# shaohua-pan/RobustCap

Measured on AMD Instinct MI355X. Metric: body-frames/sec (sig_mp fwd + FK) at batch 256, higher is better.
Workload: dtype f32; 1 GPU; synthetic 60 fps, 6 IMU + 33 keypoints, batch 256 x 1448 frames per GPU (256 bodies in total, weak scaling), confidence schedule 'mixed', seeded random weights (63.4 M params); batch_per_gpu=256, bodies_total=256, frames=1448, conf=mixed, parallelism=dp1 (sequence sharding)

## Files before the change

### robustcap_amd/csrc/rc_api.cpp

```cpp
#include "../../include/robustcap_hip.h"
#include "rc_ctx.h"

#include <algorithm>
#include <cstdio>
#include <cstdlib>
#include <cstring>
#include <map>
#include <string>
#include <thread>
#include <vector>

#define RC_SPLIT_MIN_BATCH 48
#define RC_TILE64_MIN_BATCH 192

#ifndef RC_NC1280
#define RC_NC1280 10
#endif

static thread_local std::string g_create_error;

int fail(rc_ctx* ctx, int code, const std::string& msg) {
    if (ctx) ctx->err = msg; else g_create_error = msg;
    return code;
}
// ... 152 lines not shown
    p.nt = (c->live_nt_mask >> s.net) & 1u;
    return p;
}
GemmProblem lstm_problem(const rc_ctx* c, const Stage& s, int layer) {
    const NetDev& n = c->net[s.net];
    const long long BH = (long long)c->Bp * n.H;
    GemmProblem p{};
    if (layer == 0) p.seg[0] = seg(n.x1, n.H, n.H);
    else p.seg[0] = seg(n.h, n.H, n.H, RC_PAR_DST, BH);
    p.seg[1] = seg(n.h + layer * RC_HBUF * BH, n.H, n.H, RC_PAR_SRC, BH);
    p.W = n.Wl[layer]; p.Ws = n.Wls[layer]; p.bias = n.bl[layer];
    p.hstate = n.h + layer * RC_HBUF * BH; p.cstate = n.c + layer * (long long)c->B * n.H; p.h_par_stride = BH; p.H = n.H;
    p.steps = n.steps; p.flags = s.flags ? s.flags : c->fb.flags; p.flag_bit = s.flag_bit;
    p.epi = RC_EPI_LSTM;
    int mr, nc;
    pick_tile(n.H, s.rows_hint < 0 ? c->B : s.rows_hint, &mr, &nc);
    if (s.rows_hint < 0 && c->B >= RC_TILE64_MIN_BATCH) {
        if (s.net == N6 && c->tile6[0]) { mr = c->tile6[0]; nc = c->tile6[1]; }
        if ((s.net == N3 || s.net == N7 || s.net == N8) && c->tile378[0]) { mr = c->tile378[0]; nc = c->tile378[1]; }
        if (s.net == N2 && c->tile2[0]) { mr = c->tile2[0]; nc = c->tile2[1]; }
        if (s.net == N4 && c->tile4[0]) { mr = c->tile4[0]; nc = c->tile4[1]; }
    }
    const int rows = s.rows_hint < 0 ? c->B : (s.rows_hint < c->B ? s.rows_hint : c->B);
    if (lds_problem(c, rows)) { mr = 16; nc = 8; }
    p.n_tiles = n.H / (4 * nc); p.m_tiles = (rows + 16 * mr - 1) / (16 * mr); p.Kp = 2 * n.H; p.nc = nc; p.mr = mr;
    p.nt = (c->live_nt_mask >> s.net) & 1u;
    return p;
}
GemmProblem lin2_problem(const rc_ctx* c, const Stage& s) {
    const NetDev& n = c->net[s.net];
    const long long BH = (long long)c->Bp * n.H;
    GemmProblem p = dense_problem(c, n.lin2, seg(n.h + RC_HBUF * BH, n.H, 0, RC_PAR_DST, BH), s.y, false, s.flag_bit,
                                  s.flags ? s.flags : c->fb.flags, n.steps, false);
    p.out_flags = c->fb.flags; p.out_bit = s.out_bit;
    p.nt = 1;
    return p;
}

const int kLdsRegions = 12;

int ensure_lds_pool(rc_ctx* ctx) {
    if (ctx->lds_slab) return RC_OK;
    const size_t m_tiles = ((size_t)ctx->B + 255) / 256;
    const size_t tiles = 320 * m_tiles;
    HIP_TRY(ctx, rc_alloc(ctx->lds_slab, (size_t)kLdsRegions * tiles * RC_LDS_SLAB_FLOATS));
    HIP_TRY(ctx, rc_alloc(ctx->lds_tickets, (size_t)kLdsRegions * tiles));
    HIP_TRY(ctx, hipMemset(ctx->lds_tickets.get(), 0, (size_t)kLdsRegions * tiles * sizeof(int)));
    ctx->lds_region_tiles = tiles;
    return RC_OK;
}

bool timing_pair(rc_ctx* ctx, hipEvent_t* a, hipEvent_t* b) {
    if (ctx->ev_used == ctx->ev_pool.size()) {
        std::pair<HipEvent, HipEvent> ev;
        if (hipEventCreate(rc_out(ev.first)) != hipSuccess || hipEventCreate(rc_out(ev.second)) != hipSuccess) return false;
        ctx->ev_pool.push_back(std::move(ev));
    }
    const auto& ev = ctx->ev_pool[ctx->ev_used++];
    *a = ev.first.get(); *b = ev.second.get();
    return true;
}

int build_lds_problems(rc_ctx* ctx, const std::vector<GemmProblem>& ps, const unsigned char* flags_override, float* slab, int* tickets,
                       LdsProblem* out, int max_p, int* items, size_t* tiles_out, bool resident_order) {
    std::vector<GemmProblem> ord(ps);
    auto key = [&](const GemmProblem& g) -> int {
        if (g.epi == RC_EPI_LSTM) return (resident_order && g.H == 512) ? 0 : g.Kp;
        return 1;
    };
    std::stable_sort(ord.begin(), ord.end(), [&](const GemmProblem& a, const GemmProblem& b) { return key(a) > key(b); });
    if ((int)ord.size() > max_p) return 0;
    int base = 0;
    size_t tiles = 0;
    for (size_t i = 0; i < ord.size(); ++i) {
        const GemmProblem& g = ord[i];
        LdsProblem& p = out[i];
        p = LdsProblem{};
        p.seg[0] = g.seg[0]; p.seg[1] = g.seg[1];
        p.Ws = g.Ws; p.bias = g.bias; p.hstate = g.hstate; p.cstate = g.cstate; p.steps = g.steps;
        p.flags = flags_override ? flags_override : g.flags; p.flag_bit = g.flag_bit;
        p.h_par_stride = g.h_par_stride; p.H = g.H; p.step_off = g.step_off;
        p.m_tiles = g.m_tiles; p.Qs = g.Kp / 32;
        p.epi = g.epi;
        if (g.epi == RC_EPI_LSTM) {
            p.n_tiles = g.H / 32;
            p.ksplit = ctx->lds_ksplit[g.H == 512 ? 0 : (g.H == 1024 ? 1 : 2)];
        } else {
            const long long half = (long long)(g.Kp / 32) * 256;
            p.seg[0].K = g.Kp / 2;
            p.seg[1] = p.seg[0]; p.seg[1].base = g.seg[0].base + half;
            p.alt[0] = g.alt_base; p.alt[1] = g.alt_base ? g.alt_base + half : nullptr;
            p.sel_flags = g.sel_flags; p.sel_bit = g.alt_base ? g.sel_bit : 0;
            p.out = g.out; p.ldo = g.ldo;
            p.n_tiles = g.N / 128;
            p.ksplit = 1;
        }
        p.wg_base = base;
        p.slab = slab + tiles * RC_LDS_SLAB_FLOATS; p.tickets = tickets + tiles;
        tiles += (size_t)p.n_tiles * p.m_tiles;
        base += round_up(p.n_tiles * p.m_tiles * p.ksplit, 8);
    }
    *items = base; *tiles_out = tiles;
    return (int)ord.size();
}
static void build_lds_launch(rc_ctx* ctx, const std::vector<GemmProblem>& ps, const unsigned char* flags_override, float* slab, int* tickets,
                      LdsLaunch& L, int* items, size_t* tiles_out) {
    L = LdsLaunch{};
    L.B = ctx->B;
    L.n = build_lds_problems(ctx, ps, flags_override, slab, tickets, L.p, RC_LDS_MAXP, items, tiles_out);
}

static int launch_lds(rc_ctx* ctx, const std::vector<GemmProblem>& ps_in, const unsigned char* flags_override, hipStream_t st, hipEvent_t stop, bool* launched) {
    if (int rc = ensure_lds_pool(ctx)) return rc;
    static const int replicate = std::getenv("RC_DBG_REPLICATE") ? std::atoi(std::getenv("RC_DBG_REPLICATE")) : 1;
    std::vector<GemmProblem> ps(ps_in);
    for (int r = 1; r < replicate && (int)ps.size() + (int)ps_in.size() <= RC_LDS_MAXP; ++r) ps.insert(ps.end(), ps_in.begin(), ps_in.end());
    LdsLaunch L{};
    const size_t region = ctx->lds_rot++ % kLdsRegions;
    float* slab = ctx->lds_slab.get() + region * ctx->lds_region_tiles * RC_LDS_SLAB_FLOATS;
    int* tickets = ctx->lds_tickets.get() + region * ctx->lds_region_tiles;
    int base = 0;
    size_t tiles = 0;
    build_lds_launch(ctx, ps, flags_override, slab, tickets, L, &base, &tiles);
    if (tiles > ctx->lds_region_tiles) return fail(ctx, RC_ERR_INVALID, "shared-weight launch: more tiles than its slab region holds");
    ctx->stat_lds_launches += 1;
    if (ctx->timing) {
        hipEvent_t a, b;
        if (!timing_pair(ctx, &a, &b)) return fail(ctx, RC_ERR_HIP, "hipEventCreate");
        HIP_TRY(ctx, hipEventRecord(a, st));
        rc_launch_gemm_lds(L, base, st, stop);
        if (launched && stop) *launched = true;
        HIP_TRY(ctx, hipEventRecord(b, st));
    } else {
        rc_launch_gemm_lds(L, base, st, stop);
        if (launched && stop) *launched = true;
    }
    HIP_TRY(ctx, hipGetLastError());
    return RC_OK;
}

static bool dense_items_selftest_wanted(rc_ctx* ctx, const std::vector<GemmProblem>& ps, hipStream_t st, bool fp32) {
    static const int on = std::getenv("RC_DBG_DENSE_ITEMS") ? std::atoi(std::getenv("RC_DBG_DENSE_ITEMS")) : 0;
    if (!on || !ctx->gemm_split || fp32 || ctx->B > 256 || seq_is_engine_stream(ctx, st) || (int)ps.size() > RC_RES_MAXP) return false;
    for (const GemmProblem& p : ps)
        if (!(p.epi == RC_EPI_RELU && p.out_packed && p.N % 128 == 0 && p.Kp % 128 == 0 && p.out_bit == 0 && p.out_col0 == 0 && p.seg[0].par_mode == 0)) return false;
    return true;
}
static int dense_items_selftest(rc_ctx* ctx, const std::vector<GemmProblem>& ps, const unsigned char* flags_override, hipStream_t st) {
    if (int rc = ensure_lds_pool(ctx)) return rc;
    const int n_ints = 2 + RC_RES_MAXP + 1 + 4;
    DevBuf<ResidentTick> tk_d;
    DevBuf<int> ints_d;
    HIP_TRY(ctx, rc_alloc_all(tk_d, 1, ints_d, n_ints));
    ResidentTick T{};
    std::vector<GemmProblem> q(ps);
    for (GemmProblem& p : q) p.m_tiles = 1;
    size_t tiles = 0;
    T.B = ctx->B;
    T.n = build_lds_problems(ctx, q, flags_override, ctx->lds_slab.get(), ctx->lds_tickets.get(), T.p, RC_RES_MAXP, &T.n_items, &tiles, true);
    for (int i = 0; i < RC_RES_MAXP; ++i) T.dep[i][0] = T.dep[i][1] = -1;
    const int base[2] = {0, T.n_items};
    const size_t Bp = (size_t)ctx->Bp;
    HIP_TRY(ctx, hipStreamSynchronize(st));
    for (const GemmProblem& p : ps) HIP_TRY(ctx, hipMemset(p.out, 0xff, Bp * p.N * sizeof(float)));
    HIP_TRY(ctx, hipMemcpy(tk_d.get(), &T, sizeof(T), hipMemcpyHostToDevice));
    HIP_TRY(ctx, hipMemset(ints_d.get(), 0, n_ints * sizeof(int)));
// ... 209 lines not shown
            const double x[3] = {(double)ctx->mesh_vt_h[3 * (size_t)v] - ctx->jroot_h[0], (double)ctx->mesh_vt_h[3 * (size_t)v + 1] - ctx->jroot_h[1],
                                 (double)ctx->mesh_vt_h[3 * (size_t)v + 2] - ctx->jroot_h[2]};
            for (int j = 0; j < 24; ++j) {
                const double ww = jw * ctx->mesh_w_h[(size_t)v * 24 + j];
                double* a = &acc[((size_t)k * 24 + j) * 4];
                a[0] += ww * x[0]; a[1] += ww * x[1]; a[2] += ww * x[2]; a[3] += ww;
            }
        }
    std::vector<float> kM(acc.begin(), acc.end());
    if (!ctx->mesh_kM) if (int rc = dev_alloc(ctx, &ctx->mesh_kM, (size_t)17 * 24 * 4, false)) return rc;
    HIP_TRY(ctx, hipDeviceSynchronize());
    HIP_TRY(ctx, hipMemcpy(ctx->mesh_kM, kM.data(), kM.size() * sizeof(float), hipMemcpyHostToDevice));
    ctx->fold_dirty = false;
    return RC_OK;
}

}

int check_ready(rc_ctx* ctx) {
    if (!ctx) return RC_ERR_INVALID;
    if (!ctx->have_weights) return fail(ctx, RC_ERR_STATE, "weights not finalized (rc_finalize_weights)");
    if (!ctx->have_body) return fail(ctx, RC_ERR_STATE, "body constants not set (rc_set_body)");
    return RC_OK;
}


const BodyConst* rc_ctx_body(rc_ctx* ctx) { return ctx->have_body ? ctx->body : nullptr; }
int rc_ctx_fail(rc_ctx* ctx, int code, const char* msg) { return fail(ctx, code, msg); }
static SubnetDense subnet_dense(const Dense& d) { return SubnetDense{d.W, d.Ws, d.b, d.K, d.N, d.Kp, d.Np}; }
int rc_ctx_subnet_net(rc_ctx* ctx, int ni, SubnetNet* o) {
    if (!ctx->have_weights) return RC_ERR_STATE;
    const NetDev& n = ctx->net[ni];
    o->lin1 = subnet_dense(n.lin1); o->lin2 = subnet_dense(n.lin2);
    for (int l = 0; l < 2; ++l) { o->Wl[l] = n.Wl[l]; o->Wls[l] = n.Wls[l]; o->bl[l] = n.bl[l]; }
    o->in = n.in; o->H = n.H; o->out = n.out;
    return RC_OK;
}
int rc_ctx_init_net(rc_ctx* ctx, SubnetDense out[3]) {
    if (!ctx->have_weights) return RC_ERR_STATE;
    for (int q = 0; q < 3; ++q) out[q] = subnet_dense(ctx->init[q]);
    return RC_OK;
}
int rc_ctx_net_index(const char* name) { return net_index(name); }
int rc_ctx_gemm_split(rc_ctx* ctx) { return ctx->gemm_split ? 1 : 0; }
long long rc_ctx_weights_epoch(rc_ctx* ctx) { return ctx->weights_epoch; }
SubnetOwner& rc_ctx_subnet(rc_ctx* ctx) { return ctx->subnet; }
SmplifyOwner& rc_ctx_smplify(rc_ctx* ctx) { return ctx->smplify; }
unsigned long long rc_ctx_ign_mask(rc_ctx* ctx) { return ctx->ign_mask; }


extern "C" {

int rc_default_params(int32_t live, rc_params* out) {
    if (!out) return RC_ERR_INVALID;
    std::memset(out, 0, sizeof(*out));
    out->conf_lo = live ? 0.85 : 0.7;
    out->conf_hi = live ? 0.9 : 0.8;
    out->contact_threshold = 0.7f;
    out->distance_threshold = 10.0f;
    out->height_threshold = 0.15f;
    out->tran_filter_num = live ? 0.01 : 0.05;
    out->use_flat_floor = 1; out->use_vision_updater = 1; out->use_imu_updater = 1;
    out->live = live ? 1 : 0;
    out->update_vision_freq = 30;
    out->use_reproj_opt = 0;
    out->smooth = 1.0f;
    return RC_OK;
}

int rc_create(int32_t batch, int32_t live, rc_ctx** out) {
    if (!out || batch < 1 || batch > 65535) return fail(nullptr, RC_ERR_INVALID, "rc_create: bad batch");
    int ndev = 0;
    if (hipGetDeviceCount(&ndev) != hipSuccess || ndev == 0) return fail(nullptr, RC_ERR_HIP, "rc_create: no HIP device");
    rc_ctx* ctx = new rc_ctx();
    ctx->B = batch;
    ctx->Bp = round_up(batch, RC_MT);
    (void)hipGetDevice(&ctx->dev);
    rc_default_params(live, &ctx->prm);
    ctx->gemm_split = tune_env("RC_GEMM_SPLIT", batch >= RC_SPLIT_MIN_BATCH ? 1 : 0) != 0;
    live_create(ctx);
    seq_create(ctx);
    ctx->lds_min_rows = tune_env("RC_LDS_MIN_ROWS", std::min(160, std::max(64, batch / 2)));
    ctx->lds_min_batch = tune_env("RC_LDS_MIN_BATCH", ctx->lds_min_batch);
    ctx->lds_ksplit[0] = tune_env("RC_LDS_KSPLIT_512", 1) == 1 ? 1 : 2;
    ctx->lds_ksplit[1] = tune_env("RC_LDS_KSPLIT_1024", batch <= 160 ? 1 : 2) == 1 ? 1 : 2;
    ctx->lds_ksplit[2] = tune_env("RC_LDS_KSPLIT_1280", 2) == 1 ? 1 : 2;
    ctx->tile4[0] = 4; ctx->tile4[1] = 5;
    ctx->tile6[0] = 4; ctx->tile6[1] = 8;
    ctx->tile378[0] = 4; ctx->tile378[1] = 4;
    tile_env("RC_TILE_RNN6", &ctx->tile6[0], &ctx->tile6[1]);
    tile_env("RC_TILE_S2H512", &ctx->tile378[0], &ctx->tile378[1]);
    tile_env("RC_TILE_RNN2", &ctx->tile2[0], &ctx->tile2[1]);
    tile_env("RC_TILE_RNN4", &ctx->tile4[0], &ctx->tile4[1]);
    const struct { const char* knob; int nc, H; } tiles[4] = {{"RC_TILE_RNN6", ctx->tile6[1], 1024}, {"RC_TILE_S2H512", ctx->tile378[1], 512},
                                                              {"RC_TILE_RNN2", ctx->tile2[1], 512}, {"RC_TILE_RNN4", ctx->tile4[1], 1280}};
    for (const auto& t : tiles)
        if (t.nc > 0 && t.H % (4 * t.nc) != 0) {
            rc_destroy(ctx);
            return fail(nullptr, RC_ERR_INVALID, std::string("rc_create: ") + t.knob + " tile width of " + std::to_string(4 * t.nc) +
                                                 " units does not divide H = " + std::to_string(t.H));
        }
    const size_t B = (size_t)batch, Bp = (size_t)ctx->Bp;
    int rc = RC_OK;
    FrameBuffers& fb = ctx->fb;
#define A(ptr, n) if (!rc) rc = dev_alloc(ctx, &(ptr), (n))
    for (int i = 0; i < 6 && !rc; ++i) {
        NetDev& n = ctx->net[i];
        n.in = kNets[i].in; n.H = kNets[i].H; n.out = kNets[i].out;
        n.mr = 2;
        n.nc = n.H == 1280 ? 10 : (n.H == 1024 ? 8 : 4);
        A(n.h, 2 * RC_HBUF * Bp * n.H); A(n.c, 2 * B * n.H); A(n.steps, B); A(n.x1, Bp * n.H);
        A(n.part, (size_t)(n.H / 4) * RC_LIVE_MAXB * round_up(n.out, 4));
    }
    A(ctx->hid1, Bp * 512); A(ctx->hid2, Bp * 1024); A(ctx->xtmp, Bp * 256);
    A(fb.x2, Bp * 128); A(fb.x3, Bp * 256); A(fb.x4, Bp * 256); A(fb.x6, Bp * 256); A(fb.x78, Bp * 256);
    A(fb.x4l, Bp * 256); A(fb.x6l, Bp * 256); A(fb.xi, Bp * 128);
    A(fb.vr, B * 4); A(fb.pc, B * 4); A(fb.r6d, B * 144); A(fb.contact, B * 2); A(fb.init_out, B * 2048);
    A(fb.flags, B); A(fb.flags2, B); A(fb.pend, B); A(fb.regime, B); A(fb.kconf, B); A(fb.gravity, B * 3);
    A(fb.last_pfoot, B * 6); A(fb.last_tran, B * 3); A(fb.floor, B * 33); A(fb.j_temp, B * 99);
    A(fb.has_last, B); A(fb.n_floor, B); A(fb.first_reach, B); A(fb.uv_count, B); A(fb.trace, B * 8);
    A(ctx->body, 1);
#undef A
    if (rc) { g_create_error = ctx->err; rc_destroy(ctx); return rc; }
    fb.h2 = ctx->net[N2].h; fb.c2 = ctx->net[N2].c; fb.steps2 = ctx->net[N2].steps;
    fb.h2_par_stride = (long long)Bp * 512; fb.h2_layer_stride = (long long)RC_HBUF * Bp * 512; fb.c2_layer_stride = (long long)B * 512;
    std::vector<float> g(B * 3);
    for (size_t b = 0; b < B; ++b) { g[3 * b] = -0.0029f; g[3 * b + 1] = 0.9980f; g[3 * b + 2] = -0.0273f; }
    std::vector<int> ones(B, 1);
    if (hipMemcpy(fb.gravity, g.data(), g.size() * 4, hipMemcpyHostToDevice) != hipSuccess ||
        hipMemcpy(fb.first_reach, ones.data(), B * 4, hipMemcpyHostToDevice) != hipSuccess) {
        g_create_error = "rc_create: hipMemcpy failed"; rc_destroy(ctx); return RC_ERR_HIP;
    }
    *out = ctx;
    return RC_OK;
}

int rc_destroy(rc_ctx* ctx) {
    if (!ctx) return RC_OK;
    rc_live_end(ctx);
    (void)hipDeviceSynchronize();
    delete ctx;
    return RC_OK;
}

const char* rc_last_error(const rc_ctx* ctx) { return ctx ? ctx->err.c_str() : g_create_error.c_str(); }

int rc_get_params(const rc_ctx* ctx, rc_params* out) {
    if (!ctx || !out) return RC_ERR_INVALID;
    *out = ctx->prm;
    return RC_OK;
}
int rc_set_params(rc_ctx* ctx, const rc_params* p) {
    if (!ctx || !p) return RC_ERR_INVALID;
    if (!(p->conf_hi > p->conf_lo) || p->update_vision_freq < 0) return fail(ctx, RC_ERR_INVALID, "rc_set_params: bad range");
    ctx->prm = *p;
    return RC_OK;
}

int rc_load_weight(rc_ctx* ctx, const char* key, const float* host, int64_t numel) {
    if (!ctx || !key || !host || numel <= 0) return RC_ERR_INVALID;
    std::string k(key);
    int64_t want = -1;
    for (int i = 0; i < 6 && want < 0; ++i) {
        const NetSpec& s = kNets[i];
        const std::string p = std::string(s.name) + ".";
        if (k.compare(0, p.size(), p)) continue;
// ... 601 lines not shown
```

### robustcap_amd/csrc/rc_ctx.h

```cpp
#pragma once
#include "../../include/robustcap_hip.h"
#include "rc_internal.h"

#include <map>
#include <string>
#include <utility>
#include <vector>

struct NetSpec { const char* name; int in, H, out; };
const NetSpec kNets[6] = {{"rnn2", 72, 512, 69},  {"rnn3", 141, 512, 3},   {"rnn4", 171, 1280, 69},
                          {"rnn6", 240, 1024, 3}, {"rnn7", 141, 512, 144}, {"rnn8", 141, 512, 2}};
enum { N2 = 0, N3 = 1, N4 = 2, N6 = 3, N7 = 4, N8 = 5 };

inline int round_up(int x, int m) { return (x + m - 1) / m * m; }

struct Dense {
    float* W = nullptr; float* b = nullptr;
    void* Ws = nullptr;
    float* Wrm = nullptr;
    int K = 0, N = 0, Kp = 0, Np = 0;
    int mr = 2, nc = 4;
};
struct NetDev {
    Dense lin1, lin2;
    float* Wl[2] = {nullptr, nullptr};
    void* Wls[2] = {nullptr, nullptr};
    float* bl[2] = {nullptr, nullptr};
    float* h = nullptr;
    float* c = nullptr;
    int* steps = nullptr;
    float* x1 = nullptr;
    float* part = nullptr;
    int in = 0, H = 0, out = 0;
    int nc = 4;
    int mr = 2;
};

struct rc_ctx {
    int B = 0;
    int Bp = 0;
    int dev = 0;
    rc_params prm{};
    NetDev net[6];
    Dense init[3];
    float *hid1 = nullptr, *hid2 = nullptr, *xtmp = nullptr;
    FrameBuffers fb{};
    BodyConst* body = nullptr;
    float *mesh_vt = nullptr, *mesh_w = nullptr;
    int mesh_V = 0;
    float* mesh_kM = nullptr;
    int mesh_nk = 0;
    std::vector<float> mesh_vt_h, mesh_w_h, mesh_Jr_h;
    float jroot_h[3] = {0.f, 0.f, 0.f};
    bool fold_dirty = false;
    DevBuf<float> sweep_scratch;
    size_t sweep_scratch_cap = 0;
    unsigned long long ign_mask = RC_IGN_DEFAULT;
    bool have_body = false, have_weights = false;
    long long weights_epoch = 0;
    std::map<std::string, std::vector<float>> staged;
    std::vector<DevBuf<char>> allocs;
    std::vector<std::pair<void*, size_t>> alloc_bytes;
    std::vector<DevBuf<char>> weight_allocs;
    bool alloc_weights = false;
    std::string err;
    LiveOwner live;
    SeqOwner seq;
    bool timing = false;
    int timing_mode = 1;
    std::vector<std::pair<HipEvent, HipEvent>> ev_pool;
    size_t ev_used = 0;
    double timed_ms = 0.0;
    double timed_busy_ms = 0.0;
    long long timed_launches = 0;
    bool gemm_split = false;
    bool live_launch = false;
    unsigned live_nt_mask = 63u;
    int tile6[2] = {0, 0}, tile378[2] = {0, 0}, tile2[2] = {0, 0}, tile4[2] = {0, 0};
    SmplifyOwner smplify;
    SubnetOwner subnet;
    int trace_next = 0;
    long long stat_wide_launches = 0;
    int lds_min_rows = 64;
    int lds_min_batch = 65;
    int lds_ksplit[3] = {1, 2, 2};
    DevBuf<float> lds_slab;
    DevBuf<int> lds_tickets;
    size_t lds_region_tiles = 0;
    unsigned lds_rot = 0;
    long long stat_lds_launches = 0;
    long long stat_w32_launches = 0;
};

#pragma GCC visibility push(hidden)
int fail(rc_ctx* ctx, int code, const std::string& msg);
int tune_env(const char* name, int dflt);
int check_ready(rc_ctx* ctx);
rc_params_dev dev_params(const rc_params& p);
int step_impl(rc_ctx* ctx, const FrameIO& io, uint32_t flags, hipStream_t st, bool with_tr = true, bool skip_prep = false,
              const FrameIO* next_io = nullptr, int n_live = -1);
template <typename T>
int dev_alloc(rc_ctx* ctx, T** p, size_t count, bool zero = true) {
    DevBuf<char> q;
    HIP_TRY(ctx, rc_alloc(q, count * sizeof(T)));
    if (zero) HIP_TRY(ctx, hipMemset(q.get(), 0, count * sizeof(T)));
    *p = reinterpret_cast<T*>(q.get());
    if (!ctx->alloc_weights) ctx->alloc_bytes.emplace_back(q.get(), count * sizeof(T));
    (ctx->alloc_weights ? ctx->weight_allocs : ctx->allocs).push_back(std::move(q));
    return RC_OK;
}
struct Out { float* p; int ld; int col0; bool packed; };
struct Stage {
    int net; int flag_bit; const float* x; int ldx; Out y;
    const unsigned char* flags = nullptr;
    const float* x_alt = nullptr;
    int sel_bit = 0;
    int out_bit = 0;
    int rows_hint = -1;
};
GemmSeg seg(const float* base, int ld, int K, int mode = RC_PAR_NONE, long long stride = 0);
GemmProblem dense_problem(const rc_ctx* ctx, const Dense& d, GemmSeg a, Out out, bool relu, int flag_bit, const unsigned char* flags, int* steps,
                          bool open_step);
GemmProblem lin1_problem(const rc_ctx* c, const Stage& s);
GemmProblem lstm_problem(const rc_ctx* c, const Stage& s, int layer);
GemmProblem lin2_problem(const rc_ctx* c, const Stage& s);
bool tile_env(const char* name, int* mr, int* nc);
void pick_tile(int H, int rows, int* mr, int* nc);
inline bool lds_context(const rc_ctx* c) { return c->gemm_split && c->lds_min_rows > 0 && c->B >= c->lds_min_batch; }
inline bool lds_problem(const rc_ctx* c, int rows) { return lds_context(c) && rows >= c->lds_min_rows; }
int ensure_lds_pool(rc_ctx* ctx);
bool timing_pair(rc_ctx* ctx, hipEvent_t* a, hipEvent_t* b);
int build_lds_problems(rc_ctx* ctx, const std::vector<GemmProblem>& ps, const unsigned char* flags_override, float* slab, int* tickets,
                       LdsProblem* out, int max_p, int* items, size_t* tiles_out, bool resident_order = false);
int launch_problems(rc_ctx* ctx, std::vector<GemmProblem> ps, const unsigned char* flags_override, hipStream_t st, bool fp32 = false,
                    hipEvent_t stop = nullptr, bool* launched = nullptr);
void seq_create(rc_ctx* ctx);
int seq_prepare(rc_ctx* ctx);
void seq_weights_changed(rc_ctx* ctx);
bool seq_is_engine_stream(const rc_ctx* ctx, hipStream_t st);
void live_create(rc_ctx* ctx);
void live_forget_last_frame(rc_ctx* ctx, bool rows_reset = false);
int live_discard_ahead(rc_ctx* ctx);
int mark_eager(rc_ctx* ctx, hipStream_t st);
#pragma GCC visibility pop
```

### robustcap_amd/csrc/rc_gemm_lds.hip

```cpp
#include "rc_internal.h"
#include <hip/hip_ext.h>
#include "rc_gates.h"

typedef float f32x4 __attribute__((ext_vector_type(4)));
typedef float f32x2 __attribute__((ext_vector_type(2)));
typedef unsigned int u32x4 __attribute__((ext_vector_type(4)));
typedef unsigned int u32x2 __attribute__((ext_vector_type(2)));
typedef __bf16 bf16x8 __attribute__((ext_vector_type(8)));

#ifdef RC_TRACE_TILES
__device__ unsigned long long* g_lds_trace_buf = nullptr;
__device__ unsigned long long g_lds_trace_cap = 0;
__device__ unsigned long long g_lds_trace_n = 0;
extern "C" int rc_trace_lds_set(unsigned long long* buf, unsigned long long cap_records) {
    const unsigned long long zero = 0;
    if (hipMemcpyToSymbol(HIP_SYMBOL(g_lds_trace_buf), &buf, sizeof(buf)) != hipSuccess) return -1;
    if (hipMemcpyToSymbol(HIP_SYMBOL(g_lds_trace_n), &zero, sizeof(zero)) != hipSuccess) return -1;
    return hipMemcpyToSymbol(HIP_SYMBOL(g_lds_trace_cap), &cap_records, sizeof(cap_records)) == hipSuccess ? 0 : -1;
}
#define LDS_T(i) do { if (threadIdx.x == 0) trace_t[i] = wall_clock64(); } while (0)
#define LDS_TRACE_OUT(LAST)                                                                                                  \
    do { if (threadIdx.x == 0 && g_lds_trace_buf) {                                                                          \
        const unsigned long long idx = atomicAdd(&g_lds_trace_n, 1ull);                                                      \
        if (idx < g_lds_trace_cap) { unsigned long long* r_ = g_lds_trace_buf + idx * 8;                                     \
            r_[0] = (unsigned long long)P.H | ((unsigned long long)kh0 << 16) | ((unsigned long long)P.ksplit << 20) | ((unsigned long long)(LAST) << 24) | (1ull << 32);  \
            r_[1] = __smid(); r_[2] = trace_t[0]; r_[3] = trace_t[1]; r_[4] = trace_t[2]; r_[5] = trace_t[3]; r_[6] = wall_clock64(); r_[7] = nrows; } } } while (0)
#else
#define LDS_T(i) do { } while (0)
#define LDS_TRACE_OUT(LAST) do { } while (0)
#endif

#ifndef RC_LAND
#define RC_LAND 1
#endif

namespace {

constexpr int kWaves = 8;
constexpr int kStage = 8 * 3 * 1024;
constexpr int kRing = 4;
constexpr int kPW = 3;

#define RC_MFMA(A, B, C) C = __builtin_amdgcn_mfma_f32_16x16x32_bf16(__builtin_bit_cast(bf16x8, A), __builtin_bit_cast(bf16x8, B), C, 0, 0, 0)

__device__ __forceinline__ void split_pair(const f32x2 a, unsigned& h, unsigned& m, unsigned& l) {
    const u32x2 ua = __builtin_bit_cast(u32x2, a);
    const f32x2 r1 = a - __builtin_bit_cast(f32x2, ua & 0xffff0000u);
    const u32x2 um = __builtin_bit_cast(u32x2, r1);
    const f32x2 r2 = r1 - __builtin_bit_cast(f32x2, um & 0xffff0000u);
    const u32x2 ul = __builtin_bit_cast(u32x2, r2);
    h = __builtin_amdgcn_perm(ua[1], ua[0], 0x07060302u);
    m = __builtin_amdgcn_perm(um[1], um[0], 0x07060302u);
    l = __builtin_amdgcn_perm(ul[1], ul[0], 0x07060302u);
}
__device__ __forceinline__ void split_block(const f32x4& x0, const f32x4& x1, u32x4& h, u32x4& m, u32x4& l) {
    const f32x2 a[4] = {f32x2{x0[0], x0[1]}, f32x2{x0[2], x0[3]}, f32x2{x1[0], x1[1]}, f32x2{x1[2], x1[3]}};
#pragma unroll
    for (int d = 0; d < 4; ++d) {
        unsigned hh, mm, ll;
        split_pair(a[d], hh, mm, ll);
        h[d] = hh; m[d] = mm; l[d] = ll;
    }
}

__device__ __forceinline__ void gload(f32x4& d, const float* p) { asm volatile("global_load_dwordx4 %0, %1, off" : "=v"(d) : "v"(p) : "memory"); }
__device__ __forceinline__ void gload1k(f32x4& d, const float* p) { asm volatile("global_load_dwordx4 %0, %1, off offset:1024" : "=v"(d) : "v"(p) : "memory"); }
template <int OFF>
__device__ __forceinline__ void glds(const u32x4* g, unsigned lds_) {
    const unsigned lds = __builtin_amdgcn_readfirstlane(lds_);
    unsigned keep;
    asm volatile("s_mov_b32 %0, m0\n\ts_mov_b32 m0, %2\n\ts_nop 0\n\tglobal_load_lds_dwordx4 %1, off offset:%3\n\ts_mov_b32 m0, %0"
                 : "=&s"(keep) : "v"(g), "s"(lds), "n"(OFF) : "memory");
}
template <int OFF>
__device__ __forceinline__ void dsread(u32x4& d, unsigned addr) { asm volatile("ds_read_b128 %0, %1 offset:%2" : "=v"(d) : "v"(addr), "n"(OFF) : "memory"); }
template <int N>
__device__ __forceinline__ void wait_vm() { asm volatile("s_waitcnt vmcnt(%0)" :: "n"(N) : "memory"); }

template <int CTRL>
__device__ __forceinline__ float quad(float v) {
    return __builtin_bit_cast(float, __builtin_amdgcn_mov_dpp(__builtin_bit_cast(int, v), CTRL, 0xf, 0xf, true));
}
__device__ __forceinline__ void quad_transpose(const f32x4& v, const int q, f32x4& g) {
    const bool odd = q & 1, hi = q & 2;
    const float x0 = quad<0xB1>(v[0]), x1 = quad<0xB1>(v[1]), x2 = quad<0xB1>(v[2]), x3 = quad<0xB1>(v[3]);
    const float a0 = odd ? x1 : v[0], a1 = odd ? v[1] : x0, a2 = odd ? x3 : v[2], a3 = odd ? v[3] : x2;
    const float y0 = quad<0x4E>(a0), y1 = quad<0x4E>(a1), y2 = quad<0x4E>(a2), y3 = quad<0x4E>(a3);
    g[0] = hi ? y2 : a0; g[1] = hi ? y3 : a1; g[2] = hi ? a2 : y0; g[3] = hi ? a3 : y1;
}

template <int MAXP, typename PP>
__device__ __forceinline__ bool locate(const PP Lp, const int Ln, const int item, int& pi, int& m_tile, int& n_tile, int& kh0, int& kh1) {
    pi = 0;
#pragma unroll
    for (int q = 1; q < MAXP; ++q)
        if (q < Ln && item >= Lp[q].wg_base) pi = q;
    const auto& P = Lp[pi];
    const int local = item - P.wg_base;
    const int t = P.ksplit == 2 ? local >> 1 : local;
    kh0 = P.ksplit == 2 ? (local & 1) : 0;
    kh1 = P.ksplit == 2 ? kh0 + 1 : 2;
    n_tile = t % P.n_tiles;
    m_tile = t / P.n_tiles;
    return m_tile < P.m_tiles;
}

struct HalfArgs {
    const float* pa[2];
    const u32x4* pw;
    unsigned rd0;
    unsigned my_lds;
    int Qh, Qq;
    bool primed;
};

template <int NR, bool SHORT_OK>
__device__ __forceinline__ void k_half(const HalfArgs& c, f32x4 (&acc0)[2][8], f32x4 (&acc1)[2][8]) {
    constexpr int NA = 2 * NR;
    f32x4 raw[2][2][2];
    u32x4 pl[2][3];
    u32x4 bf[2][3];
    const int Qh = c.Qh;
#define ISSUE_A(BUF, QI)                                                                                                    \
    do {                                                                                                                    \
// ... 56 lines not shown
        SLOT(0, Q, ACC); SLOT(1, Q, ACC); SLOT(2, Q, ACC); SLOT(3, Q, ACC); SLOT(4, Q, ACC); SLOT(5, Q, ACC); SLOT(6, Q, ACC); SLOT(7, Q, ACC);   \
    } while (0)

    if (c.primed) {
        ISSUE_A(0, 0); ISSUE_A(1, 1);
        wait_vm<NA>();
    } else {
        __syncthreads();
        ISSUE_A(0, 0); ISSUE_B(0); ISSUE_A(1, 1); ISSUE_B(1);
        wait_vm<NA + kPW>();
    }
    asm volatile("s_waitcnt lgkmcnt(0)\n\ts_barrier" ::: "memory");
    if constexpr (NR > 0) { dsread<0>(bf[0][0], c.rd0); dsread<1024>(bf[0][1], c.rd0); dsread<2048>(bf[0][2], c.rd0); }
#define LAND_ALL()                                                                                                          \
    do {                                                                                                                    \
        if constexpr (SHORT_OK && RC_LAND) {                                                                                \
            asm volatile("s_waitcnt vmcnt(0)\n\ts_waitcnt lgkmcnt(0)" ::: "memory");                                        \
            TIE_RAW(0); TIE_RAW(1);                                                                                         \
            if constexpr (NR > 0) asm volatile("" : "+v"(bf[0][0]), "+v"(bf[0][1]), "+v"(bf[0][2]), "+v"(bf[1][0]), "+v"(bf[1][1]), "+v"(bf[1][2])); \
        }                                                                                                                   \
    } while (0)
    LAND_ALL();
    if (SHORT_OK && c.Qq == 1) {
        ITER(0, 0, acc0); ITER(1, 1, acc1);
    } else {
        for (int q = 0; q < c.Qq; q += 2) { ITER(0, q, acc0); ITER(1, q + 1, acc0); }
        LAND_ALL();
        for (int q = c.Qq; q < Qh; q += 2) { ITER(0, q, acc1); ITER(1, q + 1, acc1); }
    }
    asm volatile("s_waitcnt vmcnt(0)\n\ts_waitcnt lgkmcnt(0)" ::: "memory");
    TIE_RAW(0); TIE_RAW(1);
    if constexpr (NR > 0) asm volatile("" : "+v"(bf[0][0]), "+v"(bf[0][1]), "+v"(bf[0][2]), "+v"(bf[1][0]), "+v"(bf[1][1]), "+v"(bf[1][2]));
#undef LAND_ALL
#undef ITER
#undef SLOT
#undef TIE_RAW
#undef ISSUE_B
#undef ISSUE_A
}

}

template <int MAXP, bool WITH_DENSE, typename PP>
__device__ __forceinline__ int lds_item(const PP Lp, const int Ln, const int LB, const int item, unsigned char* ring, int* s_rows, int* s_cnt, int* pi_out) {
#ifdef RC_TRACE_TILES
    unsigned long long trace_t[4] = {0, 0, 0, 0};
#endif
    LDS_T(0);
    int pi, m_tile, n_tile, kh0, kh1;
    const bool in_range = locate<MAXP>(Lp, Ln, item, pi, m_tile, n_tile, kh0, kh1);
    *pi_out = pi;
    if (!in_range) return 0;
#ifdef RC_SKIP_XHALF
    if (Lp[pi].epi == RC_EPI_LSTM) {
        if (Lp[pi].ksplit == 2 && kh0 == 0) return 0;
        kh0 = 1;
    }
#endif
    const auto& P = Lp[pi];
    const int B = LB;
    const int tid = threadIdx.x, lane = tid & 63;
    const int wave = __builtin_amdgcn_readfirstlane(tid >> 6);
    const int i = lane & 15, kq = lane >> 4;
    const unsigned ring0 = (unsigned)(unsigned long long)(__attribute__((address_space(3))) unsigned char*)ring;

    const int Qs = P.Qs, Qh = Qs >> 1;
    HalfArgs hc;
    hc.Qh = Qh; hc.Qq = Qh >> 1;
    hc.rd0 = ring0 + lane * 16;
    hc.my_lds = ring0 + (unsigned)wave * 3072u;
    {
        const u32x4* g_ = reinterpret_cast<const u32x4*>(P.Ws) + ((long long)(n_tile * 8 + wave) * Qs + (long long)kh0 * Qh) * 192 + lane;
        glds<0>(g_, hc.my_lds); glds<1024>(g_, hc.my_lds); glds<2048>(g_, hc.my_lds);
        glds<0>(g_ + 192, hc.my_lds + kStage); glds<1024>(g_ + 192, hc.my_lds + kStage); glds<2048>(g_ + 192, hc.my_lds + kStage);
    }
    const int lo = m_tile * 256;
    int nrows;
    if (P.flag_bit == 0) {
        nrows = min(256, B - lo);
        if (nrows <= 0) return 0;
        if (tid < 256) s_rows[tid] = lo + min(tid, nrows - 1);
        __syncthreads();
    } else {
        int total = 0;
        for (int base = 0; base < B && total < lo + 256; base += kWaves * 64) {
            const int r = base + tid;
            const bool f = r < B && (P.flags[r] & P.flag_bit);
            const unsigned long long bal = __ballot(f);
            if (lane == 0) s_cnt[wave] = __popcll(bal);
            __syncthreads();
            int woff = 0, sum = 0;
#pragma unroll
            for (int w = 0; w < kWaves; ++w) {
                const int cw = s_cnt[w];
                woff += (w < wave) ? cw : 0;
                sum += cw;
            }
            const int idx = total + woff + __popcll(bal & ((1ull << lane) - 1ull));
            if (f && idx >= lo && idx < lo + 256) s_rows[idx - lo] = r;
            total += sum;
            __syncthreads();
        }
        nrows = min(256, total - lo);
        if (nrows <= 0) return 0;
        if (tid < 256 && tid >= nrows) s_rows[tid] = s_rows[0];
        __syncthreads();
    }
    const int tile = m_tile * P.n_tiles + n_tile;
    const int nblk = (nrows + 15) >> 4;
    const int nr = wave + 8 < nblk ? 2 : (wave < nblk ? 1 : 0);
    const int row_r[2] = {s_rows[16 * wave + i], s_rows[16 * (wave + 8) + i]};
    const bool need_st = (P.seg[0].par_mode | P.seg[1].par_mode) != 0;
    const int st_r[2] = {need_st ? P.steps[row_r[0]] + P.step_off : 0, need_st ? P.steps[row_r[1]] + P.step_off : 0};

    const bool dense = WITH_DENSE && P.epi != RC_EPI_LSTM;
    f32x4 acc0[2][8], acc1[2][8];
    float* const my_slab = P.slab + ((long long)tile * 2) * 32768 + ((wave * 2) * 8 * 64 + lane) * 4;

    for (int kh = kh0; kh < kh1; ++kh) {
        const auto& sg = P.seg[kh];
#pragma unroll
        for (int r = 0; r < 2; ++r) {
            const int st = st_r[r];
            const int par = sg.par_mode == RC_PAR_SRC ? ((st - 1) % RC_HBUF) : (sg.par_mode == RC_PAR_DST ? (st % RC_HBUF) : 0);
            const float* a_base = sg.base;
            if (WITH_DENSE && P.sel_bit != 0 && !(P.sel_flags[row_r[r]] & P.sel_bit)) a_base = P.alt[kh];
            hc.pa[r] = a_base + (long long)par * sg.par_stride + rc_pk(row_r[r], 4 * kq, sg.ld);
        }
        hc.pw = reinterpret_cast<const u32x4*>(P.Ws) + ((long long)(n_tile * 8 + wave) * Qs + (long long)kh * Qh) * 192 + lane;
        hc.primed = kh == kh0;
#pragma unroll
        for (int r = 0; r < 2; ++r)
#pragma unroll
            for (int j = 0; j < 8; ++j) { acc0[r][j] = f32x4{0.f, 0.f, 0.f, 0.f}; acc1[r][j] = acc0[r][j]; }
        if (kh == kh0) LDS_T(1);
        if (nr == 2) k_half<2, WITH_DENSE>(hc, acc0, acc1);
        else if (nr == 1) k_half<1, WITH_DENSE>(hc, acc0, acc1);
        else k_half<0, WITH_DENSE>(hc, acc0, acc1);
        if (dense && kh == 1) {
            asm volatile("s_waitcnt vmcnt(0)" ::: "memory");
#pragma unroll
            for (int r = 0; r < 2; ++r)
                if (r < nr) {
#pragma unroll
                    for (int j = 0; j < 8; ++j) {
                        const f32x4 o = *reinterpret_cast<const f32x4*>(my_slab + (r * 8 + j) * 256);
                        acc0[r][j] = (o + acc0[r][j]) + acc1[r][j];
                    }
                }
        } else {
#pragma unroll
            for (int r = 0; r < 2; ++r)
#pragma unroll
                for (int j = 0; j < 8; ++j) acc0[r][j] += acc1[r][j];
        }
        if (kh == 0) {
            float* s = my_slab;
#pragma unroll
            for (int r = 0; r < 2; ++r)
                if (r < nr) {
#pragma unroll
                    for (int j = 0; j < 8; ++j) *reinterpret_cast<f32x4*>(s + (r * 8 + j) * 256) = acc0[r][j];
                }
        }
    }

    LDS_T(2);
    const int q = i & 3, u = i >> 2;
    int rr_[2], r2_[2], dst_[2];
    float c_prev[2][8], bias[8];
    const bool finisher = P.ksplit != 2 || kh0 == 1;
    if (dense) {
#pragma unroll
        for (int r = 0; r < 2; ++r) {
            rr_[r] = 16 * (wave + 8 * r) + 4 * kq + q;
            r2_[r] = s_rows[rr_[r] < nrows ? rr_[r] : 0];
            dst_[r] = 0;
        }
#pragma unroll
        for (int j = 0; j < 8; ++j) bias[j] = P.bias[n_tile * 128 + 16 * j + i];
    } else if (finisher) {
#pragma unroll
        for (int r = 0; r < 2; ++r) {
            rr_[r] = 16 * (wave + 8 * r) + 4 * kq + q;
            r2_[r] = s_rows[rr_[r] < nrows ? rr_[r] : 0];
            dst_[r] = (P.steps[r2_[r]] + P.step_off) % RC_HBUF;
#pragma unroll
            for (int j = 0; j < 8; ++j) c_prev[r][j] = P.cstate[(long long)r2_[r] * P.H + n_tile * 32 + j * 4 + u];
        }
#pragma unroll
        for (int j = 0; j < 8; ++j) bias[j] = P.bias[n_tile * 128 + 16 * j + i];
    }
#ifdef RC_SKIP_XHALF
    if (false) {
#else
    if (P.ksplit == 2) {
#endif
        if (kh0 == 0) {
            asm volatile("s_waitcnt vmcnt(0)" ::: "memory");
            __syncthreads();
            if (tid == 0) {
                __builtin_amdgcn_fence(__ATOMIC_RELEASE, "agent");
                asm volatile("s_waitcnt vmcnt(0)" ::: "memory");
                __hip_atomic_store(&P.tickets[tile], 1, __ATOMIC_RELAXED, __HIP_MEMORY_SCOPE_AGENT);
            }
            LDS_T(3); LDS_TRACE_OUT(0);
            return 0;
        }
        if (tid == 0) {
            const unsigned long long t_give_up = wall_clock64() + 200000000ull;
            while (__hip_atomic_load(&P.tickets[tile], __ATOMIC_RELAXED, __HIP_MEMORY_SCOPE_AGENT) == 0) {
                __builtin_amdgcn_s_sleep(8);
                if (wall_clock64() > t_give_up) __builtin_trap();
            }
            __hip_atomic_store(&P.tickets[tile], 0, __ATOMIC_RELAXED, __HIP_MEMORY_SCOPE_AGENT);
            __builtin_amdgcn_fence(__ATOMIC_ACQUIRE, "agent");
        }
        __syncthreads();
    } else {
        asm volatile("s_waitcnt vmcnt(0)" ::: "memory");
    }
    LDS_T(3);
#pragma unroll
    for (int r = 0; r < 2; ++r) {
        if (r >= nr) continue;
        const bool ok = rr_[r] < nrows;
        if (dense) {
#pragma unroll
            for (int j = 0; j < 8; ++j) {
                f32x4 v = acc0[r][j];
                v[0] += bias[j]; v[1] += bias[j]; v[2] += bias[j]; v[3] += bias[j];
                f32x4 g;
                quad_transpose(v, q, g);
                g[0] = fmaxf(g[0], 0.0f); g[1] = fmaxf(g[1], 0.0f); g[2] = fmaxf(g[2], 0.0f); g[3] = fmaxf(g[3], 0.0f);
                if (ok) *reinterpret_cast<f32x4*>(&P.out[rc_pk(r2_[r], n_tile * 128 + 16 * j + 4 * u, P.ldo)]) = g;
            }
            continue;
        }
        f32x4 o[8];
#pragma unroll
        for (int j = 0; j < 8; ++j) o[j] = *reinterpret_cast<const f32x4*>(my_slab + (r * 8 + j) * 256);
#pragma unroll
        for (int j = 0; j < 8; ++j) {
            f32x4 v = o[j] + acc0[r][j];
            v[0] += bias[j]; v[1] += bias[j]; v[2] += bias[j]; v[3] += bias[j];
            f32x4 g;
            quad_transpose(v, q, g);
            float cn, hn;
            rc_lstm_cell(g[0], g[1], g[2], g[3], c_prev[r][j], cn, hn);
            if (ok) {
                const int unit = n_tile * 32 + j * 4 + u;
                P.cstate[(long long)r2_[r] * P.H + unit] = cn;
                P.hstate[(long long)dst_[r] * P.h_par_stride + rc_pk(r2_[r], unit, P.H)] = hn;
            }
        }
    }
    LDS_TRACE_OUT(1);
    return 1;
}

__global__ __launch_bounds__(kWaves * 64, 1) void rc_gemm_lds_kernel(const LdsLaunch L) {
    __shared__ __attribute__((aligned(1024))) unsigned char ring[kRing * kStage];
    __shared__ int s_rows[256];
    __shared__ int s_cnt[kWaves];
    int pi;
    (void)lds_item<RC_LDS_MAXP, false, const LdsProblem*>(L.p, L.n, L.B, (int)blockIdx.x, ring, s_rows, s_cnt, &pi);
}

__device__ __forceinline__ int ld_agent(const int* p) { return __hip_atomic_load(p, __ATOMIC_RELAXED, __HIP_MEMORY_SCOPE_AGENT); }

__device__ __forceinline__ void resident_wait(const ResidentArgs& R, const __attribute__((address_space(4))) ResidentTick* T, const int k, const int pi) {
    if (threadIdx.x == 0) {
        const unsigned long long give_up = wall_clock64() + R.spin_bound;
        const int prev_items = k >= 2 ? R.item_base[k - 1] - R.item_base[k - 2] : 0;
        bool ok = false;
        for (;;) {
            ok = ld_agent(R.flag_tail) >= (T->need_tail[pi] ? k : k - 1);
            if (ok && k >= 2) ok = ld_agent(R.tick_done + (k - 2)) >= prev_items;
#pragma unroll
            for (int d = 0; d < 2; ++d)
                if (ok && T->dep[pi][d] >= 0) ok = ld_agent(R.done + (long long)(k - 1) * RC_RES_MAXP + T->dep[pi][d]) >= T->dep_items[pi][d];
            if (ok || ld_agent(R.abort) != 0) break;
            if (wall_clock64() > give_up) { __hip_atomic_store(R.abort, 1, __ATOMIC_RELAXED, __HIP_MEMORY_SCOPE_AGENT); break; }
            __builtin_amdgcn_s_sleep(4);
        }
        __builtin_amdgcn_fence(__ATOMIC_ACQUIRE, "agent");
    }
    __syncthreads();
}

__global__ __launch_bounds__(kWaves * 64, 1) void rc_gemm_resident_kernel(const ResidentArgs R) {
    __shared__ __attribute__((aligned(1024))) unsigned char ring[kRing * kStage];
    __shared__ int s_rows[256];
    __shared__ int s_cnt[kWaves];
    __shared__ int s_item;
    const int total = R.item_base[R.n_ticks];
    int k = 0;
#ifdef RC_RES_PROF
    __shared__ unsigned long long s_prof[6];
    enum { p_wait = 0, p_item = 1, p_n = 2, p_rel = 3, p_grab = 4, p_t = 5 };
    if (threadIdx.x == 0) { for (int i = 0; i < 5; ++i) s_prof[i] = 0; s_prof[p_t] = wall_clock64(); }
#define RES_STAMP(ACC) do { if (threadIdx.x == 0) { const unsigned long long n_ = wall_clock64(); s_prof[ACC] += n_ - s_prof[p_t]; s_prof[p_t] = n_; } } while (0)
#else
#define RES_STAMP(ACC) do { } while (0)
#endif
    for (;;) {
        if (threadIdx.x == 0) s_item = __hip_atomic_fetch_add(R.head, 1, __ATOMIC_RELAXED, __HIP_MEMORY_SCOPE_AGENT);
        __syncthreads();
        const int g = __builtin_amdgcn_readfirstlane(s_item);
#ifdef RC_RES_PROF
        if (g >= total) {
            if (threadIdx.x == 0) {
                unsigned long long* prof = (unsigned long long*)(((unsigned long long)(R.abort + 1) + 7ull) & ~7ull);
                for (int i = 0; i < 5; ++i) atomicAdd(prof + i, s_prof[i]);
            }
            return;
        }
        RES_STAMP(p_grab);
#endif
        if (g >= total) return;
        while (g >= R.item_base[k + 1]) ++k;
        typedef const __attribute__((address_space(4))) ResidentTick* TickC;
        const TickC T = (TickC)(unsigned long long)(R.ticks + k);
        const int item = g - R.item_base[k];
        int pi = 0;
        for (int q = 1; q < T->n; ++q) if (item >= T->p[q].wg_base) pi = q;
        resident_wait(R, T, k, pi);
        RES_STAMP(p_wait);
        typedef const __attribute__((address_space(4))) LdsProblem* ProbC;
        (void)lds_item<RC_RES_MAXP, true, ProbC>(T->p, T->n, T->B, item, ring, s_rows, s_cnt, &pi);
        RES_STAMP(p_item);
#ifdef RC_RES_PROF
        if (threadIdx.x == 0) s_prof[p_n] += 1;
#endif
        asm volatile("s_waitcnt vmcnt(0)" ::: "memory");
        __syncthreads();
        if (threadIdx.x == 0) {
            __builtin_amdgcn_fence(__ATOMIC_RELEASE, "agent");
            asm volatile("s_waitcnt vmcnt(0)" ::: "memory");
            __hip_atomic_fetch_add(R.done + (long long)k * RC_RES_MAXP + pi, 1, __ATOMIC_RELAXED, __HIP_MEMORY_SCOPE_AGENT);
            __hip_atomic_fetch_add(R.tick_done + k, 1, __ATOMIC_RELAXED, __HIP_MEMORY_SCOPE_AGENT);
            asm volatile("s_waitcnt vmcnt(0)" ::: "memory");
        }
        RES_STAMP(p_rel);
    }
}

__global__ void rc_flag_set_kernel(int* flag, int value) {
    __hip_atomic_store(flag, value, __ATOMIC_RELEASE, __HIP_MEMORY_SCOPE_AGENT);
}
__global__ void rc_flag_wait_kernel(const int* counter, int target, int* abort, unsigned long long spin_bound) {
    const unsigned long long give_up = wall_clock64() + spin_bound;
    while (ld_agent(counter) < target && ld_agent(abort) == 0) {
        if (wall_clock64() > give_up) { __hip_atomic_store(abort, 1, __ATOMIC_RELAXED, __HIP_MEMORY_SCOPE_AGENT); break; }
        __builtin_amdgcn_s_sleep(8);
    }
    __builtin_amdgcn_fence(__ATOMIC_ACQUIRE, "agent");
}

void rc_launch_gemm_resident(const ResidentArgs& R, int workgroups, hipStream_t s) {
    hipLaunchKernelGGL(rc_gemm_resident_kernel, dim3(workgroups), dim3(kWaves * 64), 0, s, R);
}
void rc_launch_flag_set(int* flag, int value, hipStream_t s) { hipLaunchKernelGGL(rc_flag_set_kernel, dim3(1), dim3(1), 0, s, flag, value); }
void rc_launch_flag_wait(const int* counter, int target, int* abort, unsigned long long spin_bound, hipStream_t s) {
    hipLaunchKernelGGL(rc_flag_wait_kernel, dim3(1), dim3(1), 0, s, counter, target, abort, spin_bound);
}

void rc_launch_gemm_lds(const LdsLaunch& L, int total_wg, hipStream_t s, hipEvent_t stop) {
    const dim3 g(total_wg), b(kWaves * 64);
    if (stop) hipExtLaunchKernelGGL(rc_gemm_lds_kernel, g, b, 0, s, nullptr, stop, 0, L);
    else hipLaunchKernelGGL(rc_gemm_lds_kernel, g, b, 0, s, L);
}
```

### robustcap_amd/csrc/rc_internal.h

```cpp
#pragma once
#include <hip/hip_runtime.h>
#include <stdint.h>
#include <memory>
#include <string>
#include <type_traits>

#define RC_MT 32
#define RC_NT 64
#ifndef RC_NW
#define RC_NW 4
#endif
#define RC_KC 16
#define RC_KALIGN 128
#define RC_HBUF 3
#define RC_MAX_PROB 14

__host__ __device__ inline long long rc_pk(long long row, int k, int ld) {
    return (row >> 4) * (16ll * ld) + (long long)(k >> 4) * 256 + ((k >> 2) & 3) * 64 + (row & 15) * 4 + (k & 3);
}

enum { RC_EPI_DENSE = 0, RC_EPI_RELU = 1, RC_EPI_LSTM = 2 };
enum { RC_PAR_NONE = 0, RC_PAR_SRC = 1, RC_PAR_DST = 2 };

#define RC_ROW_VIS 1u
#define RC_ROW_PC 2u
#define RC_ROW_UPD 4u
#define RC_ROW_REACH 8u
#define RC_ROW_MASK 16u
#define RC_ROW2_TR 1u
#define RC_ROW2_M4 2u
#define RC_ROW2_M6 4u
#define RC_ROW2_FLUSH 8u
#define RC_ROW2_VALID 16u

struct GemmSeg {
    const float* base;
    long long par_stride;
    int ld;
    int K;
    int par_mode;
    int pad_;
};

struct GemmProblem {
    GemmSeg seg[2];
    const float* W;
    const void* Ws;
    const float* bias;
    float* out;
    float* hstate;
    float* cstate;
    int* steps;
    const unsigned char* flags;
    const float* alt_base;
    const unsigned char* sel_flags;
    const unsigned char* out_flags;
    long long h_par_stride;
    int ldo, N, H;
    int out_col0, out_packed;
    int sel_bit, out_bit;
    int flag_bit;
    int epi;
    int open_step;
    int n_tiles, m_tiles, wg_base, Kp;
    int nc;
    int mr;
    int trace_base;
    int nt;
    int step_off;
};

struct GemmLaunch {
    int n;
    int B;
    int split;
    int live;
    GemmProblem p[RC_MAX_PROB];
};

#define RC_TICK_PROB 24

#define RC_LDS_MAXP 12
#define RC_LDS_SLAB_FLOATS 65536
struct LdsProblem {
    GemmSeg seg[2];
    const void* Ws;
    const float* bias;
    float* hstate;
    float* cstate;
    const int* steps;
    const unsigned char* flags;
    float* slab;
    int* tickets;
    long long h_par_stride;
    int H, flag_bit, n_tiles, m_tiles, wg_base, Qs, step_off, ksplit;
    float* out;
    const float* alt[2];
    const unsigned char* sel_flags;
    int epi, ldo, sel_bit, pad_;
};
struct LdsLaunch {
    int n, B;
    LdsProblem p[RC_LDS_MAXP];
};
#define RC_RES_MAXP 20
void rc_launch_gemm_lds(const LdsLaunch& L, int total_wg, hipStream_t s, hipEvent_t stop = nullptr);

struct ResidentTick {
    int n, B;
    LdsProblem p[RC_RES_MAXP];
    int n_items;
    int dep[RC_RES_MAXP][2];
    int dep_items[RC_RES_MAXP][2];
    int need_tail[RC_RES_MAXP];
};
struct ResidentArgs {
    const ResidentTick* ticks;
    const int* item_base;
    int n_ticks;
    int* head;
    int* done;
    int* tick_done;
    const int* flag_tail;
    int* abort;
    unsigned long long spin_bound;
};
void rc_launch_gemm_resident(const ResidentArgs& R, int workgroups, hipStream_t s);
void rc_launch_flag_set(int* flag, int value, hipStream_t s);
void rc_launch_flag_wait(const int* counter, int target, int* abort, unsigned long long spin_bound, hipStream_t s);

struct BodyConst {
    int parent[24];
    int level[24];
    float bone[24][3];
    float jrest[24][3];
    float jroot[3];
    float w33[33][24];
    float v33[33][3];
    int override_joint[33];
    int nchild[24];
    int child[24][4];
};

struct FrameBuffers {
    float *x2, *x3, *x4, *x6, *x78, *x4l, *x6l, *xi;
    float *vr, *pc, *r6d, *contact;
    float *init_out;
    unsigned char* flags;
    unsigned char* flags2;
    unsigned char* pend;
    unsigned char* regime;
    double* kconf;
    float* gravity;
    float *last_pfoot, *last_tran, *floor, *j_temp;
    int *has_last, *n_floor, *first_reach, *uv_count;
    int* trace;
    float *h2, *c2;
    int* steps2;
    long long h2_par_stride, h2_layer_stride, c2_layer_stride;
    int* frame;
    int* wsteps;
};

struct WavePrep {
    const int* frame_at;
    int* steps[6];
    const float *cx4l, *cx6l;
    int first_tick;
    int t0;
};
struct WaveTail {
    int on;
    int t_last;
    float *x4l, *x6l;
    unsigned char* flags2;
    int* wsteps;
    int *steps4, *steps6;
    float *cx4l, *cx6l;
};

struct FrameIO {
    const float *j2d, *acc, *ori, *first_tran;
// ... 315 lines not shown
```

Measured before the change: 1.264 million body-frames/s.

## Gather active rows as contiguous 16-row blocks in LDS GEMM when block count allows

Measured after the change: 1.283 million body-frames/s (median of 6 runs). +1.5%, better.

```diff
diff --git a/robustcap_amd/csrc/rc_api.cpp b/robustcap_amd/csrc/rc_api.cpp
--- a/robustcap_amd/csrc/rc_api.cpp
+++ b/robustcap_amd/csrc/rc_api.cpp
@@ -258,6 +258,7 @@
         p.h_par_stride = g.h_par_stride; p.H = g.H; p.step_off = g.step_off;
         p.m_tiles = g.m_tiles; p.Qs = g.Kp / 32;
         p.epi = g.epi;
+        p.block_pick = ctx->lds_block_pick && ctx->B <= 256 && g.m_tiles == 1 ? 1 : 0;
         if (g.epi == RC_EPI_LSTM) {
             p.n_tiles = g.H / 32;
             p.ksplit = ctx->lds_ksplit[g.H == 512 ? 0 : (g.H == 1024 ? 1 : 2)];
@@ -633,6 +634,7 @@
     seq_create(ctx);
     ctx->lds_min_rows = tune_env("RC_LDS_MIN_ROWS", std::min(160, std::max(64, batch / 2)));
     ctx->lds_min_batch = tune_env("RC_LDS_MIN_BATCH", ctx->lds_min_batch);
+    ctx->lds_block_pick = tune_env("RC_LDS_BLOCK_PICK", 1) != 0;
     ctx->lds_ksplit[0] = tune_env("RC_LDS_KSPLIT_512", 1) == 1 ? 1 : 2;
     ctx->lds_ksplit[1] = tune_env("RC_LDS_KSPLIT_1024", batch <= 160 ? 1 : 2) == 1 ? 1 : 2;
     ctx->lds_ksplit[2] = tune_env("RC_LDS_KSPLIT_1280", 2) == 1 ? 1 : 2;
diff --git a/robustcap_amd/csrc/rc_ctx.h b/robustcap_amd/csrc/rc_ctx.h
--- a/robustcap_amd/csrc/rc_ctx.h
+++ b/robustcap_amd/csrc/rc_ctx.h
@@ -84,6 +84,7 @@
     int lds_min_rows = 64;
     int lds_min_batch = 65;
     int lds_ksplit[3] = {1, 2, 2};
+    bool lds_block_pick = true;
     DevBuf<float> lds_slab;
     DevBuf<int> lds_tickets;
     size_t lds_region_tiles = 0;
diff --git a/robustcap_amd/csrc/rc_gemm_lds.hip b/robustcap_amd/csrc/rc_gemm_lds.hip
--- a/robustcap_amd/csrc/rc_gemm_lds.hip
+++ b/robustcap_amd/csrc/rc_gemm_lds.hip
@@ -40,6 +40,9 @@
 constexpr int kStage = 8 * 3 * 1024;
 constexpr int kRing = 4;
 constexpr int kPW = 3;
+constexpr int kCnt = 3 * kWaves;
+constexpr int kRowIdle = (int)0x80000000u;
+constexpr int kRowMask = 0x7fffffff;
 
 #define RC_MFMA(A, B, C) C = __builtin_amdgcn_mfma_f32_16x16x32_bf16(__builtin_bit_cast(bf16x8, A), __builtin_bit_cast(bf16x8, B), C, 0, 0, 0)
 
@@ -262,26 +265,57 @@
         if (tid < 256) s_rows[tid] = lo + min(tid, nrows - 1);
         __syncthreads();
     } else {
-        int total = 0;
+        int total = 0, nact = 0;
+        bool blocks = false;
+        const bool pick = P.block_pick != 0 && B <= 256;
         for (int base = 0; base < B && total < lo + 256; base += kWaves * 64) {
             const int r = base + tid;
             const bool f = r < B && (P.flags[r] & P.flag_bit);
             const unsigned long long bal = __ballot(f);
-            if (lane == 0) s_cnt[wave] = __popcll(bal);
+            if (lane == 0) {
+                int cnt = __popcll(bal);
+                if (pick) {
+                    const unsigned lo32 = (unsigned)bal, hi32 = (unsigned)(bal >> 32);
+                    const unsigned bm = ((lo32 & 0xffffu) ? 1u : 0u) | ((lo32 >> 16) ? 2u : 0u) | ((hi32 & 0xffffu) ? 4u : 0u) | ((hi32 >> 16) ? 8u : 0u);
+                    cnt |= (int)(bm << 16);
+                    s_cnt[kWaves + 2 * wave] = (int)lo32;
+                    s_cnt[kWaves + 2 * wave + 1] = (int)hi32;
+                }
+                s_cnt[wave] = cnt;
+            }
             __syncthreads();
             int woff = 0, sum = 0;
 #pragma unroll
             for (int w = 0; w < kWaves; ++w) {
-                const int cw = s_cnt[w];
+                const int cw = s_cnt[w] & 0xffff;
                 woff += (w < wave) ? cw : 0;
                 sum += cw;
             }
-            const int idx = total + woff + __popcll(bal & ((1ull << lane) - 1ull));
-            if (f && idx >= lo && idx < lo + 256) s_rows[idx - lo] = r;
+            unsigned amask = 0;
+            if (pick && sum > 0) {
+#pragma unroll
+                for (int w = 0; w < 4; ++w) amask |= (unsigned)(s_cnt[w] >> 16) << (4 * w);
+                nact = __popc(amask);
+                blocks = ((nact + 3) >> 2) == ((((sum + 15) >> 4) + 3) >> 2);
+            }
+            if (blocks) {
+                if (tid < 16 * nact) {
+                    int blk = 0, seen = 0;
+#pragma unroll
+                    for (int j = 0; j < 16; ++j) {
+                        if ((amask >> j) & 1u) { if (seen == (tid >> 4)) blk = j; ++seen; }
+                    }
+                    const unsigned w16 = (unsigned)s_cnt[kWaves + (blk >> 1)] >> (16 * (blk & 1));
+                    s_rows[tid] = (16 * blk + (tid & 15)) | (((w16 >> (tid & 15)) & 1u) ? 0 : kRowIdle);
+                }
+            } else {
+                const int idx = total + woff + __popcll(bal & ((1ull << lane) - 1ull));
+                if (f && idx >= lo && idx < lo + 256) s_rows[idx - lo] = r;
+            }
             total += sum;
             __syncthreads();
         }
-        nrows = min(256, total - lo);
+        nrows = blocks ? 16 * nact : min(256, total - lo);
         if (nrows <= 0) return 0;
         if (tid < 256 && tid >= nrows) s_rows[tid] = s_rows[0];
         __syncthreads();
@@ -289,9 +323,11 @@
     const int tile = m_tile * P.n_tiles + n_tile;
     const int nblk = (nrows + 15) >> 4;
     const int nr = wave + 8 < nblk ? 2 : (wave < nblk ? 1 : 0);
-    const int row_r[2] = {s_rows[16 * wave + i], s_rows[16 * (wave + 8) + i]};
+    const int e_r[2] = {s_rows[16 * wave + i], s_rows[16 * (wave + 8) + i]};
+    const int row_r[2] = {e_r[0] & kRowMask, e_r[1] & kRowMask};
+    const int row_c[2] = {min(row_r[0], B - 1), min(row_r[1], B - 1)};
     const bool need_st = (P.seg[0].par_mode | P.seg[1].par_mode) != 0;
-    const int st_r[2] = {need_st ? P.steps[row_r[0]] + P.step_off : 0, need_st ? P.steps[row_r[1]] + P.step_off : 0};
+    const int st_r[2] = {need_st ? (e_r[0] >= 0 ? P.steps[row_c[0]] + P.step_off : 1) : 0, need_st ? (e_r[1] >= 0 ? P.steps[row_c[1]] + P.step_off : 1) : 0};
 
     const bool dense = WITH_DENSE && P.epi != RC_EPI_LSTM;
     f32x4 acc0[2][8], acc1[2][8];
@@ -304,7 +340,7 @@
             const int st = st_r[r];
             const int par = sg.par_mode == RC_PAR_SRC ? ((st - 1) % RC_HBUF) : (sg.par_mode == RC_PAR_DST ? (st % RC_HBUF) : 0);
             const float* a_base = sg.base;
-            if (WITH_DENSE && P.sel_bit != 0 && !(P.sel_flags[row_r[r]] & P.sel_bit)) a_base = P.alt[kh];
+            if (WITH_DENSE && P.sel_bit != 0 && !(P.sel_flags[row_c[r]] & P.sel_bit)) a_base = P.alt[kh];
             hc.pa[r] = a_base + (long long)par * sg.par_stride + rc_pk(row_r[r], 4 * kq, sg.ld);
         }
         hc.pw = reinterpret_cast<const u32x4*>(P.Ws) + ((long long)(n_tile * 8 + wave) * Qs + (long long)kh * Qh) * 192 + lane;
@@ -354,7 +390,9 @@
 #pragma unroll
         for (int r = 0; r < 2; ++r) {
             rr_[r] = 16 * (wave + 8 * r) + 4 * kq + q;
-            r2_[r] = s_rows[rr_[r] < nrows ? rr_[r] : 0];
+            const int e_ = s_rows[rr_[r] < nrows ? rr_[r] : 0];
+            if (e_ < 0) rr_[r] = 256;
+            r2_[r] = min(e_ & kRowMask, B - 1);
             dst_[r] = 0;
         }
 #pragma unroll
@@ -363,7 +401,9 @@
 #pragma unroll
         for (int r = 0; r < 2; ++r) {
             rr_[r] = 16 * (wave + 8 * r) + 4 * kq + q;
-            r2_[r] = s_rows[rr_[r] < nrows ? rr_[r] : 0];
+            const int e_ = s_rows[rr_[r] < nrows ? rr_[r] : 0];
+            if (e_ < 0) rr_[r] = 256;
+            r2_[r] = min(e_ & kRowMask, B - 1);
             dst_[r] = (P.steps[r2_[r]] + P.step_off) % RC_HBUF;
 #pragma unroll
             for (int j = 0; j < 8; ++j) c_prev[r][j] = P.cstate[(long long)r2_[r] * P.H + n_tile * 32 + j * 4 + u];
@@ -442,7 +482,7 @@
 __global__ __launch_bounds__(kWaves * 64, 1) void rc_gemm_lds_kernel(const LdsLaunch L) {
     __shared__ __attribute__((aligned(1024))) unsigned char ring[kRing * kStage];
     __shared__ int s_rows[256];
-    __shared__ int s_cnt[kWaves];
+    __shared__ int s_cnt[kCnt];
     int pi;
     (void)lds_item<RC_LDS_MAXP, false, const LdsProblem*>(L.p, L.n, L.B, (int)blockIdx.x, ring, s_rows, s_cnt, &pi);
 }
@@ -472,7 +512,7 @@
 __global__ __launch_bounds__(kWaves * 64, 1) void rc_gemm_resident_kernel(const ResidentArgs R) {
     __shared__ __attribute__((aligned(1024))) unsigned char ring[kRing * kStage];
     __shared__ int s_rows[256];
-    __shared__ int s_cnt[kWaves];
+    __shared__ int s_cnt[kCnt];
     __shared__ int s_item;
     const int total = R.item_base[R.n_ticks];
     int k = 0;
diff --git a/robustcap_amd/csrc/rc_internal.h b/robustcap_amd/csrc/rc_internal.h
--- a/robustcap_amd/csrc/rc_internal.h
+++ b/robustcap_amd/csrc/rc_internal.h
@@ -97,7 +97,8 @@
     float* out;
     const float* alt[2];
     const unsigned char* sel_flags;
-    int epi, ldo, sel_bit, pad_;
+    int epi, ldo, sel_bit;
+    int block_pick;
 };
 struct LdsLaunch {
     int n, B;
```
